# kyutai-labs/pocket-tts

Measured on AMD Instinct MI355X. Metric: audio-seconds/sec (xRT), 100M en model, whole job over all GPUs, higher is better.
Workload: dtype f32

## Files before the change

include/ptts.h:

```cpp
#ifndef PTTS_H_
#define PTTS_H_

#include <stdint.h>

#ifdef __cplusplus
extern "C" {
#endif

#define PTTS_ABI_VERSION 1

typedef struct ptts_engine ptts_engine;
typedef struct ptts_lm_state ptts_lm_state;
typedef struct ptts_mimi_state ptts_mimi_state;
typedef struct ptts_graph ptts_graph;
typedef struct ptts_resampler ptts_resampler;
typedef struct ptts_stretcher ptts_stretcher;
typedef struct ptts_pitcher ptts_pitcher;
typedef struct ptts_leveler ptts_leveler;
typedef struct ptts_loudnorm ptts_loudnorm;
typedef struct ptts_tone ptts_tone;
typedef struct ptts_dynamics ptts_dynamics;
typedef struct ptts_encoder ptts_encoder;
typedef struct ptts_flac ptts_flac;

// ... 39 lines not shown
int ptts_lm_state_copy(ptts_lm_state *dst, const ptts_lm_state *src, void *stream);
int ptts_lm_state_copy_row(ptts_lm_state *dst, int32_t row, const ptts_lm_state *src, void *stream);
int ptts_lm_state_copy_row_from(ptts_lm_state *dst, int32_t row, const ptts_lm_state *src, int32_t src_row, void *stream);
int ptts_lm_state_offsets(ptts_lm_state *s, int32_t *h_offsets, void *stream);

int ptts_lm_prefill(ptts_engine *e, ptts_lm_state *s, const float *d_emb, int32_t t, void *stream);
int ptts_lm_prefill_ragged(ptts_engine *e, ptts_lm_state *s, const float *d_emb, const int32_t *h_len, int32_t t_max,
                           void *stream);
int ptts_embed_tokens(ptts_engine *e, const float *d_table, int32_t n_bins, const int64_t *d_tokens, int64_t n,
                      float *d_out, void *stream);

int ptts_lm_decode_step(ptts_engine *e, ptts_lm_state *s, const float *d_latent_in, const float *d_noise,
                        int32_t lsd_steps, float eos_threshold, float *d_latent_out, float *d_eos_logit,
                        uint8_t *d_is_eos, void *stream);
int ptts_lm_set_noise(ptts_lm_state *s, float temp, uint64_t seed);
int ptts_lm_state_set_row_seed(ptts_lm_state *s, int32_t row, uint64_t seed, void *stream);
int ptts_lm_state_clear_row_seed(ptts_lm_state *s, int32_t row, void *stream);
int ptts_lm_state_set_row_sampling(ptts_lm_state *s, int32_t row, float temp, float noise_clamp, float eos_threshold,
                                   void *stream);
int ptts_lm_state_clear_row_sampling(ptts_lm_state *s, int32_t row, void *stream);
int ptts_lm_state_reserve_row_lsd(ptts_lm_state *s, int32_t K, void *stream);
int ptts_lm_state_set_row_lsd(ptts_lm_state *s, int32_t row, int32_t n, void *stream);
int ptts_lm_state_clear_row_lsd(ptts_lm_state *s, int32_t row, void *stream);
const float *ptts_lm_latent_ptr(ptts_lm_state *s);

int ptts_mimi_state_create(ptts_engine *e, int32_t batch, ptts_mimi_state **out);
void ptts_mimi_state_destroy(ptts_mimi_state *s);
int ptts_mimi_state_reset(ptts_mimi_state *s, void *stream);
int ptts_mimi_state_reset_row(ptts_mimi_state *s, int32_t row, void *stream);
int ptts_lm_state_set_row_active(ptts_lm_state *s, int32_t row, int32_t active, void *stream);
int ptts_mimi_set_pcm_i16(ptts_mimi_state *s, int16_t *d_pcm_i16);
int ptts_resampler_create(ptts_engine *e, int32_t batch, const int32_t *h_up, const int32_t *h_down, const int32_t *h_taps,
                          int32_t n_rates, const float *h_tables, int64_t n_table_floats, ptts_resampler **out);
void ptts_resampler_destroy(ptts_resampler *rs);
int ptts_resampler_set_row(ptts_resampler *rs, int32_t row, int32_t rate_index, void *stream);
int ptts_resample_frame(ptts_resampler *rs, const float *d_pcm_in, void *out, int32_t is_i16, void *stream);
int ptts_mimi_set_resampler(ptts_mimi_state *s, ptts_resampler *rs, void *out, int32_t is_i16);
int ptts_stretcher_create(ptts_engine *e, int32_t batch, const int32_t *h_plans, int32_t n_plans, const float *h_windows,
                          int64_t n_window_floats, ptts_stretcher **out);
void ptts_stretcher_destroy(ptts_stretcher *ts);
int ptts_stretcher_set_row(ptts_stretcher *ts, int32_t row, int32_t plan_index, void *stream);
int ptts_stretcher_set_row_drain(ptts_stretcher *ts, int32_t row, int32_t on, void *stream);
int ptts_stretch_frame(ptts_stretcher *ts, const float *d_in, void *out, int32_t is_i16, int32_t *d_delta, void *stream);
int ptts_mimi_set_stretcher(ptts_mimi_state *s, ptts_stretcher *ts, float *d_in, void *out, int32_t is_i16);
int ptts_pitcher_create(ptts_engine *e, int32_t batch, const int32_t *h_plans, int32_t n_plans, const float *h_windows,
                        int64_t n_window_floats, const float *h_tables, int64_t n_table_floats, ptts_pitcher **out);
// ... 158 lines not shown
```

pocket_tts_amd/_lib.py:

```python

from __future__ import annotations

import ctypes as C
import os
import subprocess
from pathlib import Path

PKG = Path(__file__).resolve().parent
LIB_PATH = PKG / "libptts.so"
SRC = PKG / "csrc" / "ptts.hip"
HEADER = PKG.parent / "include" / "ptts.h"

HIPCC_FLAGS = ["--offload-arch=gfx950", "-O3", "-std=c++17", "-ffp-contract=on", "-Wno-unused-value", "-Wno-unused-result",
               "-shared", "-fPIC"]


class PttsConfig(C.Structure):
    _fields_ = [
        ("d_model", C.c_int32), ("num_heads", C.c_int32), ("num_layers", C.c_int32), ("ff_dim", C.c_int32),
        ("ldim", C.c_int32), ("flow_dim", C.c_int32), ("flow_depth", C.c_int32), ("max_period", C.c_float),
        ("m_dim", C.c_int32), ("m_heads", C.c_int32), ("m_layers", C.c_int32), ("m_ff", C.c_int32),
        ("m_context", C.c_int32), ("m_max_period", C.c_float),
        ("n_filters", C.c_int32), ("ratios", C.c_int32 * 3), ("kernel_size", C.c_int32),
        ("res_kernel_size", C.c_int32), ("last_kernel_size", C.c_int32), ("compress", C.c_int32),
# ... 46 lines not shown
    "ptts_create_from_file": (C.c_int, [C.c_char_p, C.c_int32, C.POINTER(_P)]),
    "ptts_destroy": (None, [_P]),
    "ptts_lm_state_create": (C.c_int, [_P, C.c_int32, C.c_int32, C.POINTER(_P)]),
    "ptts_lm_state_destroy": (None, [_P]),
    "ptts_lm_state_reset": (C.c_int, [_P, _P]),
    "ptts_lm_state_import": (C.c_int, [_P, C.c_int32, _P, C.c_int32, C.c_int32, _P]),
    "ptts_lm_state_export": (C.c_int, [_P, C.c_int32, _P, C.c_int32, _P]),
    "ptts_lm_state_copy": (C.c_int, [_P, _P, _P]),
    "ptts_lm_state_copy_row": (C.c_int, [_P, C.c_int32, _P, _P]),
    "ptts_lm_state_copy_row_from": (C.c_int, [_P, C.c_int32, _P, C.c_int32, _P]),
    "ptts_lm_state_offsets": (C.c_int, [_P, C.POINTER(C.c_int32), _P]),
    "ptts_lm_prefill": (C.c_int, [_P, _P, _P, C.c_int32, _P]),
    "ptts_lm_prefill_ragged": (C.c_int, [_P, _P, _P, _P, C.c_int32, _P]),
    "ptts_lm_decode_step": (C.c_int, [_P, _P, _P, _P, C.c_int32, C.c_float, _P, _P, _P, _P]),
    "ptts_lm_latent_ptr": (_P, [_P]),
    "ptts_lm_set_noise": (C.c_int, [_P, C.c_float, C.c_uint64]),
    "ptts_lm_state_set_row_sampling": (C.c_int, [_P, C.c_int32, C.c_float, C.c_float, C.c_float, _P]),
    "ptts_lm_state_clear_row_sampling": (C.c_int, [_P, C.c_int32, _P]),
    "ptts_lm_state_set_row_seed": (C.c_int, [_P, C.c_int32, C.c_uint64, _P]),
    "ptts_lm_state_clear_row_seed": (C.c_int, [_P, C.c_int32, _P]),
    "ptts_lm_state_reserve_row_lsd": (C.c_int, [_P, C.c_int32, _P]),
    "ptts_lm_state_set_row_lsd": (C.c_int, [_P, C.c_int32, C.c_int32, _P]),
    "ptts_lm_state_clear_row_lsd": (C.c_int, [_P, C.c_int32, _P]),
    "ptts_profile_start": (C.c_int, [_P]),
    "ptts_profile_stop": (C.c_int64, [_P, C.c_char_p, C.c_int64]),
    "ptts_mimi_state_create": (C.c_int, [_P, C.c_int32, C.POINTER(_P)]),
    "ptts_mimi_state_destroy": (None, [_P]),
    "ptts_mimi_state_reset": (C.c_int, [_P, _P]),
    "ptts_mimi_decode": (C.c_int, [_P, _P, _P, _P, _P]),
    "ptts_encode_voice": (C.c_int, [_P, _P, C.c_int64, _P, _P, C.POINTER(C.c_int32), _P]),
    "ptts_graph_capture_lm_step": (C.c_int, [_P, _P, _P, C.c_int32, C.c_float, _P, _P, _P, C.POINTER(_P)]),
    "ptts_graph_capture_mimi": (C.c_int, [_P, _P, _P, _P, C.POINTER(_P)]),
    "ptts_mimi_decode_tr": (C.c_int, [_P, _P, _P, _P, _P]),
    "ptts_mimi_decode_seanet": (C.c_int, [_P, _P, _P, _P]),
    "ptts_graph_capture_mimi_tr": (C.c_int, [_P, _P, _P, C.POINTER(_P)]),
    "ptts_graph_capture_mimi_tr_pair": (C.c_int, [_P, _P, _P, _P, C.POINTER(_P)]),
    "ptts_graph_capture_mimi_seanet": (C.c_int, [_P, _P, _P, C.POINTER(_P)]),
    "ptts_graph_capture_pipelined": (C.c_int, [_P, _P, _P, _P, C.c_int32, C.c_float, _P, _P, _P, _P, _P, C.POINTER(_P)]),
    "ptts_graph_launch": (C.c_int, [_P, _P]),
    "ptts_graph_destroy": (None, [_P]),
    "ptts_mimi_state_reset_row": (C.c_int, [_P, C.c_int32, _P]),
    "ptts_lm_state_set_row_active": (C.c_int, [_P, C.c_int32, C.c_int32, _P]),
    "ptts_mimi_set_pcm_i16": (C.c_int, [_P, _P]),
    "ptts_resampler_create": (C.c_int, [_P, C.c_int32, C.POINTER(C.c_int32), C.POINTER(C.c_int32), C.POINTER(C.c_int32),
                                        C.c_int32, C.POINTER(C.c_float), C.c_int64, C.POINTER(_P)]),
    "ptts_resampler_destroy": (None, [_P]),
# ... 162 lines not shown
```

pocket_tts_amd/csrc/ptts.hip:

```cpp
#include "ptts_host.h"
#include "ptts_flow.h"
#include "ptts_bf16.h"
#include "ptts_lm.h"

#include <algorithm>
#include <array>
#include <cmath>
#include <cstdio>
#include <cstring>

static thread_local std::string g_err;
int fail(int code, const std::string &msg) {
  g_err = msg;
  return code;
}
static thread_local std::string g_launch_err;
bool launch_err_pending() { return !g_launch_err.empty(); }
int take_launch_err() {
  std::string m;
  m.swap(g_launch_err);
  return fail(-4, m);
}
void note_launch_err(const std::string &msg) { if (g_launch_err.empty()) g_launch_err = msg; }

// ... 1097 lines not shown
  hipStream_t st = S(s->e, stream);
  ENGINE_LOCK(s->e);
  set_int_kernel<<<1, 64, 0, st>>>(s->seed_on + row, 1, 0);
  LAUNCHCHK();
  return 0;
}

static int ensure_flow(ptts_engine *e, ptts_lm_state *s, int steps, hipStream_t st);

extern "C" int ptts_lm_state_reserve_row_lsd(ptts_lm_state *s, int32_t K, void *stream) {
  if (!s || K < 1 || K > 64) return fail(-1, "reserve_row_lsd: capacity must be in [1, 64]");
  ptts_engine *e = s->e;
  ENGINE_LOCK(e);
  HIPCHK(hipSetDevice(e->device));
  if (s->n_graphs > 0) return fail(-1, "reserve_row_lsd: the state has captured graphs (they hold its flow buffers): reserve before capturing");
  K = std::max(K, (int32_t)s->lsd_cap);
  CHK(ensure_flow(e, s, K, S(e, stream)));
  CHK(prepare_lsd_pack(e, K));
  s->lsd_tab = e->tpack[K];
  s->lsd_cap = K;
  return 0;
}

extern "C" int ptts_lm_state_set_row_lsd(ptts_lm_state *s, int32_t row, int32_t n, void *stream) {
  if (!s || row < 0 || row >= s->B) return fail(-1, "set_row_lsd: row out of range");
  if (s->lsd_cap < 1) return fail(-1, "set_row_lsd: the state has no per-row LSD capacity (ptts_lm_state_reserve_row_lsd)");
  if (n < 1 || n > s->lsd_cap) return fail(-1, "set_row_lsd: lsd_decode_steps must be in [1, " + std::to_string(s->lsd_cap) + "]");
  hipStream_t st = S(s->e, stream);
  ENGINE_LOCK(s->e);
  set_int_kernel<<<1, 64, 0, st>>>(s->lsd_n + row, 1, n);
  LAUNCHCHK();
  return 0;
}

extern "C" int ptts_lm_state_clear_row_lsd(ptts_lm_state *s, int32_t row, void *stream) {
  if (!s || row < 0 || row >= s->B) return fail(-1, "clear_row_lsd: row out of range");
  hipStream_t st = S(s->e, stream);
  ENGINE_LOCK(s->e);
  set_int_kernel<<<1, 64, 0, st>>>(s->lsd_n + row, 1, 0);
  LAUNCHCHK();
  return 0;
}

extern "C" int ptts_profile_start(ptts_engine *e) {
  if (!e) return fail(-1, "null engine");
  ENGINE_LOCK(e);
// ... 22 lines not shown
  e->prof.recs.clear();
  std::string out;
  char line[512];
  for (auto &k : order) {
    auto &v = agg[k];
    snprintf(line, sizeof line, "%s %s %.0f %.6f %.0f %.0f\n", k.first.empty() ? "-" : k.first.c_str(), k.second.c_str(), v[0], v[1], v[2], v[3]);
    out += line;
  }
  if ((int64_t)out.size() + 1 > capacity) return fail(-1, "profile buffer too small");
  memcpy(h_out, out.c_str(), out.size() + 1);
  return (int64_t)out.size();
}


static bool flow_cluster_ok(const ptts_engine *e, const ptts_lm_state *s) {
  const ptts_config &c = e->cfg;
  const int FDF = c.flow_dim / 16, LF = c.ldim / 16;
  if (!e->opt_flow_cluster || c.flow_depth > FLOW_MAX_DEPTH || FDF > 64 || LF > FDF) return false;
  const int kpw = cdiv(std::max(FDF, LF), FLOW_WORKERS);
  if (kpw != 1 && kpw != 2 && kpw != 4) return false;
  if (!e->input_proj.bias || !e->fin.bias) return false;
  for (auto &r : e->res) if (!r.l0.bias || !r.l2.bias) return false;
  return FDF <= std::min(e->opt_flow_max_cus, e->n_cus);
}
static int ensure_flow(ptts_engine *e, ptts_lm_state *s, int steps, hipStream_t st) {
  if (steps <= s->flow_steps) return 0;
  if (s->n_graphs > 0)
    return fail(-1, "lsd_decode_steps grows beyond what this state's captured graphs were built for: destroy the graphs first "
                    "(they hold the old AdaLN / exchange buffers)");
  const ptts_config &c = e->cfg;
  const int FDF = c.flow_dim / 16;
  static const int rt_env = [] { const char *v = getenv("PTTS_FLOW_RT"); return v ? atoi(v) : 1; }();
  s->flow_rt = (rt_env == 2 && s->MT >= 2) ? 2 : 1;
  s->flow_ng = cdiv(s->MT, s->flow_rt);
  HIPCHK(hipStreamSynchronize(st));
  HIPCHK(hipStreamSynchronize(e->stream));
  AllocScope alloc_scope(st);
  hipFree(s->mod); hipFree(s->fexch); hipFree(s->fflags);
  s->mod = nullptr; s->fexch = nullptr; s->fflags = nullptr;
  const size_t rt = (size_t)s->MT * 256;
  const int nph = steps * (2 * c.flow_depth + 2);
  CHK(dallocT(nullptr, &s->mod, (size_t)steps * rt * e->adaln.NT));
  CHK(dallocT(nullptr, &s->fexch, (size_t)s->flow_ng * nph * s->flow_rt * FDF * 256));
  CHK(dallocT(nullptr, &s->fflags, (size_t)s->flow_ng * nph * FDF));
  HIPCHK(hipStreamSynchronize(st));
  s->flow_steps = steps;
  return 0;
}

template <int RT, bool ROWLSD>
static void launch_flow_rt(hipStream_t st, const FlowArgs &fa, int kpw) {
  const dim3 grid(fa.NCL * fa.FDF), block(FLOW_THREADS);
  switch (kpw) {
    case 1: flow_cluster_kernel<RT, 1, ROWLSD><<<grid, block, 0, st>>>(fa); break;
    case 2: flow_cluster_kernel<RT, 2, ROWLSD><<<grid, block, 0, st>>>(fa); break;
    default: flow_cluster_kernel<RT, 4, ROWLSD><<<grid, block, 0, st>>>(fa); break;
  }
}

static int flow_steps_of(const ptts_lm_state *s, int lsd_steps) { return std::max(lsd_steps, s->lsd_cap); }

static void launch_flow_cluster(hipStream_t st, ptts_engine *e, ptts_lm_state *s, int lsd_steps, float *d_latent_out) {
  const ptts_config &c = e->cfg;
  const int FDF = c.flow_dim / 16, LF = c.ldim / 16;
  FlowArgs fa;
  memset(&fa, 0, sizeof fa);
  fa.MT = s->MT; fa.M = s->B; fa.NG = s->flow_ng; fa.NCL = std::max(1, std::min(s->flow_ng, std::min(e->opt_flow_max_cus, e->n_cus) / FDF)); fa.FDF = FDF; fa.LF = LF; fa.AF = e->adaln.NT;
  const bool rowlsd = s->lsd_cap > 0;
  fa.depth = c.flow_depth; fa.steps = rowlsd ? flow_steps_of(s, lsd_steps) : lsd_steps; fa.ldim = c.ldim;
  fa.w_in = e->input_proj.w; fa.b_in = e->input_proj.bias;
  for (int r = 0; r < c.flow_depth; ++r) {
    fa.w_l0[r] = e->res[r].l0.w; fa.b_l0[r] = e->res[r].l0.bias;
    fa.w_l2[r] = e->res[r].l2.w; fa.b_l2[r] = e->res[r].l2.bias;
    fa.ln_w[r] = e->res[r].ln_w; fa.ln_b[r] = e->res[r].ln_b;
  }
  fa.w_fin = e->fin.w; fa.b_fin = e->fin.bias;
  fa.mod = s->mod; fa.mod_step = (long)s->MT * 256 * e->adaln.NT;
  fa.latfm = s->latfm;
  fa.lat = s->lat; fa.lat_out1 = s->lat_prev; fa.lat_out2 = d_latent_out;
  fa.inv_steps = 1.0f / (float)lsd_steps;
  fa.exch = s->fexch; fa.flags = s->fflags; fa.ctr = s->rng_ctr; fa.err = s->ferr;
  fa.row_n = rowlsd ? s->lsd_n : nullptr; fa.row_ndef = lsd_steps;
  const double wbytes = 4.0 * 256 * ((double)FDF * LF + 2.0 * c.flow_depth * FDF * FDF + (double)LF * FDF);
  const double flops = 2.0 * s->B * 256.0 * ((double)FDF * LF + 2.0 * c.flow_depth * FDF * FDF + (double)LF * FDF) * lsd_steps;
  ProfScope ps(st, std::string(rowlsd ? "flow_cluster_rowlsd@" : "flow_cluster@") + std::to_string((long)fa.NCL * FDF * FLOW_THREADS),
               lsd_steps * (wbytes + 4.0 * s->B * 16.0 * e->adaln.NT), flops);
  const int kpw = cdiv(std::max(FDF, LF), FLOW_WORKERS);
  s->coop_wgs = std::max(s->coop_wgs, fa.NCL * FDF);
  if (rowlsd) {
    if (s->flow_rt == 2) launch_flow_rt<2, true>(st, fa, kpw);
    else launch_flow_rt<1, true>(st, fa, kpw);
  } else {
    if (s->flow_rt == 2) launch_flow_rt<2, false>(st, fa, kpw);
    else launch_flow_rt<1, false>(st, fa, kpw);
  }
}


static constexpr int kLmMaxWGs = 256;
static bool lm_cluster_ok(const ptts_engine *e, const ptts_lm_state *s) {
  if (!e->opt_lm_cluster || !e->lm_table) return false;
  if (e->cfg.d_model / 16 > std::min(kLmMaxWGs, e->n_cus)) return false;
  if (s->n_pre > 0) return false;
  return (double)s->kv_plane() * 4.0 < 2.0e9;
}
static int ensure_lm_cluster(ptts_engine *e, ptts_lm_state *s, hipStream_t st) {
  if (s->lexch || !e->lm_table) return 0;
  const ptts_config &c = e->cfg;
  const int DF = c.d_model / 16, FFF = c.ff_dim / 16;
  AllocScope alloc_scope(st);
  CHK(dallocT(nullptr, &s->lexch, (size_t)s->MT * c.num_layers * (4 * DF + FFF) * 256));
// ... 205 lines not shown
  GemmArgs a;
  if (lm_cluster_ok(e, s) && s->lexch) {
    SITE("lm.cluster");
    launch_lm_cluster(st, e, s, sc);
  } else {
    lm_layers(st, e, s, sc, B, 1, true);
  }
  SITE("flow.head");
  a = mk_gemm(e->head, sc.x, DF, MT, B);
  a.epi = EPI_HEAD; a.Y = s->ce; a.YF = FDF; a.head_nt = FDF; a.eos_thr = eos_thr;
  a.eos_on = s->samp_on; a.eos_row = s->samp_eos;
  a.eos_logit = s->eos_logit; a.is_eos = s->is_eos;
  a.eos_logit2 = d_eos_logit; a.is_eos2 = d_is_eos;
  a.tail_offset = s->offset; a.tail_ctr = s->rng_ctr; a.tail_rctr = s->seed_ctr; a.tail_active = s->active;
  const bool silu_in_head = lsd_steps == 1 && s->lsd_cap == 0;
  if (silu_in_head) { a.act = ACT_SILU; a.prevec = tcomb; }
  launch_gemm(st, a, PRE_LNFOLD);
  const int AF = e->adaln.NT;
  const bool rowlsd = s->lsd_cap > 0;
  const int nit = rowlsd ? flow_steps_of(s, lsd_steps) : lsd_steps;
  auto row_lsd = [&](GemmArgs &g, int i) {
    g.row_n = s->lsd_n; g.row_tab = s->lsd_tab; g.row_ndef = lsd_steps; g.row_i = i;
  };
  if (flow_cluster_ok(e, s) && nit <= s->flow_steps) {
    if (rowlsd) {
      SITE("flow.adaln");
      a = mk_gemm(e->adaln, s->ce, FDF, MT, B);
      a.prevec = tcomb; a.Y = s->mod; a.YF = AF;
      row_lsd(a, 0);
      a.row_nz = nit; a.row_zstride = (long)MT * 256 * AF;
      launch_gemm(st, a, PRE_ADDSILU_ROW);
    } else {
      for (int i = 0; i < lsd_steps; ++i) {
        SITE("flow.adaln");
        a = mk_gemm(e->adaln, s->ce, FDF, MT, B);
        a.prevec = tcomb + (size_t)i * FD; a.Y = s->mod + (size_t)i * MT * 256 * AF; a.YF = AF;
        launch_gemm(st, a, silu_in_head ? PRE_NONE : PRE_ADDSILU);
      }
    }
    SITE("flow.cluster");
    launch_flow_cluster(st, e, s, lsd_steps, d_latent_out);
    s->latfm_noise = true;
  } else {
  s->latfm_noise = false;
  for (int i = 0; i < nit; ++i) {
    SITE("flow.adaln");
    a = mk_gemm(e->adaln, s->ce, FDF, MT, B);
// ... 434 lines not shown
```

pocket_tts_amd/csrc/ptts_debug.hip:

```cpp
#include "ptts_bf16.h"
#include "ptts_host.h"

#include <algorithm>
#include <cstring>


static constexpr unsigned kDbgUnwritten = 0x7fc00000u;
static constexpr unsigned kDbgGuard = 0x7fa5a5a5u;
static constexpr long kDbgGuardFloats = 16384;
static constexpr long kAttnGuard = 16 * 64;

static __global__ void dbg_guard_kernel(const unsigned *p, long n, unsigned pattern, int *bad) {
  const long i = (long)blockIdx.x * blockDim.x + threadIdx.x;
  if (i < n && p[i] != pattern) atomicOr(bad, 1);
}
__device__ __forceinline__ float dbg_e4m3(uint8_t b) { return __builtin_amdgcn_cvt_f32_fp8((int)b, 0); }
static __global__ void dbg_from_codec_kernel(const void *src, float *dst, int M, int N, int KB, int fmt) {
  const long i = (long)blockIdx.x * blockDim.x + threadIdx.x;
  if (i >= (long)M * N) return;
  const int m = i / N, n = i - (long)m * N;
  const size_t o = fmh_off(m, n & ~3, KB) + (n & 3);
  dst[i] = fmt == 0 ? (float)((const __bf16 *)src)[o] : dbg_e4m3(((const uint8_t *)src)[o]);
}

// ... 22 lines not shown
  int *bad = nullptr;
  CHK(dallocT(&scr, &bad, 1));
  for (const void *g : guards) dbg_guard_kernel<<<cdiv(n, 256), 256, 0, st>>>((const unsigned *)g, n, kDbgGuard, bad);
  LAUNCHCHK();
  int h_bad = 0;
  HIPCHK(hipMemcpyAsync(&h_bad, bad, sizeof(int), hipMemcpyDeviceToHost, st));
  HIPCHK(hipStreamSynchronize(st));
  if (h_bad) return fail(-6, what);
  return 0;
}

extern "C" int64_t ptts_debug_read(ptts_engine *e, void *state, int32_t is_mimi, const char *name, float *d_out,
                                   int64_t capacity, int32_t *rows, int32_t *cols, void *stream) {
  hipStream_t st = S(e, stream);
  const ptts_config &c = e->cfg;
  const float *src = nullptr;
  int M = 0, K = 0, F = 0;
  std::string n(name);
  if (!is_mimi) {
    ptts_lm_state *s = (ptts_lm_state *)state;
    if (n == "x") { src = s->dec.x; M = s->B; K = c.d_model; }
    else if (n == "ce") { src = s->ce; M = s->B; K = c.flow_dim; }
    else if (n == "fx") { src = s->fx; M = s->B; K = c.flow_dim; }
    else if (n == "prefill_x") { src = s->pre.x; M = s->pre.MT * 16; K = c.d_model; }
    else if (n == "noise") {
      if (!s->latfm_noise) return fail(-1, "debug_read: noise is only kept by steps that ran the flow cluster");
      src = s->latfm; M = s->B; K = c.ldim;
    }
    else return fail(-1, "unknown buffer " + n);
    F = K / 16;
  } else {
    ptts_mimi_state *s = (ptts_mimi_state *)state;
    const int par = (s->h_frame - 1) & 1;
    const int B = s->B;
    if (n == "upsample") { src = s->u0; M = B * 16; K = c.m_dim; }
    else if (n == "dec_tr") { src = s->tr_out.slot((s->h_frame - 1) & (s->tr_out.slots - 1)); M = B * 16; K = c.m_dim; }
    else if (n.compare(0, 11, "dec_tr_slot") == 0) {
      const int k = atoi(n.c_str() + 11);
      if (n.size() != 12 || k < 0 || k >= s->tr_out.slots) return fail(-1, "unknown buffer " + n);
      src = s->tr_out.slot(k); M = B * 16; K = c.m_dim;
    }
    else if (n == "seanet0") { src = s->a0.slot(par); M = B * 16; K = 8 * c.n_filters; }
    else if (n == "tr_attn") { src = s->ao; M = B * 16; K = c.m_dim; }
    else if (n == "tr_resid") { src = s->u; M = B * 16; K = c.m_dim; }
    else if (n == "tr_ff") { src = s->ff; M = B * 16; K = c.m_ff; }
    else if (n == "seanet11") {
// ... 586 lines not shown
```

pocket_tts_amd/csrc/ptts_flow.h:

```cpp
#pragma once
#include "ptts_kernels.h"

#define FLOW_MAX_DEPTH 12
#define FLOW_WORKERS 8
#define FLOW_THREADS (64 * (FLOW_WORKERS + 1))
#define FLOW_SPIN_LIMIT 400000u

typedef unsigned u32x4 __attribute__((ext_vector_type(4)));
typedef unsigned long long u64;

struct FlowArgs {
  int MT, M, NG, NCL, FDF, LF, AF, depth, steps, ldim;
  const float *w_in, *b_in;
  const float *w_l0[FLOW_MAX_DEPTH], *b_l0[FLOW_MAX_DEPTH], *w_l2[FLOW_MAX_DEPTH], *b_l2[FLOW_MAX_DEPTH];
  const float *ln_w[FLOW_MAX_DEPTH], *ln_b[FLOW_MAX_DEPTH];
  const float *w_fin, *b_fin;
  const float *mod;
  long mod_step;
  const float *latfm;
  float *lat, *lat_out1, *lat_out2;
  float inv_steps;
  float *exch;
  u64 *flags;
  const int *ctr;
  int *err;
  const int *row_n;
  int row_ndef;
};

__device__ __forceinline__ __amdgpu_buffer_rsrc_t flow_rsrc(const void *p) {
  return __builtin_amdgcn_make_buffer_rsrc(const_cast<void *>(p), 0, 0x7ffffff0, 0x00020000);
}
__device__ __forceinline__ f32x4 flow_ld_sc1(__amdgpu_buffer_rsrc_t r, unsigned byte_off) {
  return __builtin_bit_cast(f32x4, __builtin_amdgcn_raw_buffer_load_b128(r, (int)byte_off, 0, 16));
}
__device__ __forceinline__ void flow_st_sc1(__amdgpu_buffer_rsrc_t r, unsigned byte_off, f32x4 v) {
  __builtin_amdgcn_raw_buffer_store_b128(__builtin_bit_cast(u32x4, v), r, (int)byte_off, 0, 16);
}

__device__ __forceinline__ bool flow_wait(const u64 *f, int np, u64 epoch, int lane, int *err) {
  for (unsigned spins = 0;; ++spins) {
    const u64 v = lane < np ? __hip_atomic_load(f + lane, __ATOMIC_RELAXED, __HIP_MEMORY_SCOPE_AGENT) : epoch;
    if (__all(v == epoch)) return true;
    if (spins > FLOW_SPIN_LIMIT) {
      if (lane == 0) atomicExch(err, 1);
      return false;
    }
    __builtin_amdgcn_s_sleep(2);
  }
}

template <int RT, int KPW, bool ROWLSD = false>
__global__ __launch_bounds__(FLOW_THREADS) void flow_cluster_kernel(FlowArgs a) {
  const int lane = threadIdx.x & 63, wave = threadIdx.x >> 6;
  const int FDF = a.FDF, LF = a.LF;
  const int cl = blockIdx.x / a.FDF, j = blockIdx.x % a.FDF;
  const bool coord = wave == FLOW_WORKERS;
  const int PPS = 2 * a.depth + 2, NPH = a.steps * PPS;
  __shared__ f32x4 red[FLOW_WORKERS][RT][64];
  __shared__ float st[FLOW_WORKERS][RT][16][2];
// ... 202 lines not shown
          latv[t] = latv[t] + s * a.inv_steps;
        }
        out = latv[t];
        const int m = 16 * (mt0 + t) + (lane & 15);
        if (last && j < LF && mt0 + t < a.MT && m < a.M) {
          const size_t o = (size_t)m * a.ldim + 16 * j + 4 * (lane >> 4);
          *(f32x4 *)(a.lat + o) = out;
          if (a.lat_out1) *(f32x4 *)(a.lat_out1 + o) = out;
          if (a.lat_out2) *(f32x4 *)(a.lat_out2 + o) = out;
        }
      }
      if (publish) flow_st_sc1(rs, ((unsigned)((p * RT + t) * FDF + j) * 64u + lane) * 16u, out);
    }
    if (publish) {
      asm volatile("s_waitcnt vmcnt(0)" ::: "memory");
      if (lane == 0) __hip_atomic_store(fl + (size_t)p * FDF + j, ebase | (u64)(p + 1), __ATOMIC_RELAXED, __HIP_MEMORY_SCOPE_AGENT);
    }
    e_bias = n_bias;
#pragma unroll
    for (int t = 0; t < RT; ++t) e_gate[t] = n_gate[t];
  }
  }
}
```

pocket_tts_amd/csrc/ptts_host.h:

```cpp
#pragma once
#include "ptts_kernels.h"
#include "ptts_ext.h"

#include <array>
#include <map>
#include <mutex>
#include <string>
#include <vector>

#include "../../include/ptts.h"

#pragma GCC visibility push(hidden)

int fail(int code, const std::string &msg);
#define HIPCHK(x)                                                                                      \
  do {                                                                                                 \
    hipError_t e_ = (x);                                                                               \
    if (e_ != hipSuccess)                                                                              \
      return fail(-2, std::string(#x) + ": " + hipGetErrorString(e_) + " @" + std::to_string(__LINE__)); \
  } while (0)
#define CHK(x)            \
  do {                    \
    int r_ = (x);         \
    if (r_ < 0) return r_; \
// ... 121 lines not shown
  int quant_flags = 0;
};
#define ENGINE_LOCK(e) std::lock_guard<std::recursive_mutex> lock_((e)->mu)

struct Scratch {
  float *x = nullptr, *h = nullptr, *ao = nullptr, *ff = nullptr, *q = nullptr, *part = nullptr, *rope = nullptr;
  int MT = 0, QB = 0, splits_cap = 0;
};

struct ptts_lm_state {
  ptts_engine *e;
  int B, cap, MT;
  float *kv = nullptr;
  int *offset = nullptr;
  int *qlen = nullptr;
  std::vector<int> h_off;
  Scratch dec, pre;
  float *xlat, *c, *ce, *mod, *latfm, *fx, *fh, *f1;
  float *fstat = nullptr;
  float *fexch = nullptr;
  unsigned long long *fflags = nullptr;
  int *ferr = nullptr;
  int flow_steps = 0, flow_rt = 1, flow_ng = 1;
  int lsd_cap = 0;
  const float *lsd_tab = nullptr;
  int *lsd_n = nullptr;
  KvPrefix *d_pre = nullptr;
  std::vector<KvPrefix> h_pre;
  std::vector<ptts_lm_state *> pre_owner;
  int casc_mode = -1;
  int n_pre = 0;
  int borrowers = 0;
  bool zombie = false;
  int n_graphs = 0;
  int coop_wgs = 0;
  float *lexch = nullptr;
  unsigned long long *lflags = nullptr;
  float *lat, *lat_prev;
  float *eos_logit;
  uint8_t *is_eos;
  float rng_std = 0.f;
  unsigned long long rng_seed = 0;
  int *rng_ctr = nullptr;
  int *samp_on = nullptr;
  f32x4 *samp_noise = nullptr;
  float *samp_eos = nullptr;
// ... 138 lines not shown
```

pocket_tts_amd/engine.py:

```python

from __future__ import annotations

import ctypes as C
import numbers
import os
import weakref

import numpy as np
import torch

from . import _lib
from .config import Config
from .weights import mimi_encode_spec, state_dict_spec


def _ptr(t: torch.Tensor | None):
    return None if t is None else C.c_void_p(t.data_ptr())


def make_ptts_config(cfg: Config) -> _lib.PttsConfig:
    t, m, sn = cfg.flow_lm.transformer, cfg.mimi.transformer, cfg.mimi.seanet
    if len(sn.ratios) != 3:
        raise ValueError("SEANet decoder with 3 upsampling stages expected")
    pc = _lib.PttsConfig()
# ... 71 lines not shown
    def set_row_sampling(self, row: int, temp: float, noise_clamp: float | None = None, eos_threshold: float = -4.0):
        clamp = 0.0 if noise_clamp is None else float(noise_clamp)
        _lib.check(self.engine.lib.ptts_lm_state_set_row_sampling(self.handle, row, float(temp), clamp,
                                                                  float(eos_threshold), self.engine._sp))

    def clear_row_sampling(self, row: int):
        _lib.check(self.engine.lib.ptts_lm_state_clear_row_sampling(self.handle, row, self.engine._sp))

    def set_row_seed(self, row: int, seed: int):
        _lib.check(self.engine.lib.ptts_lm_state_set_row_seed(self.handle, row, check_seed(seed, bits=64),
                                                              self.engine._sp))

    def clear_row_seed(self, row: int):
        _lib.check(self.engine.lib.ptts_lm_state_clear_row_seed(self.handle, row, self.engine._sp))

    def reserve_row_lsd(self, K: int):
        _lib.check(self.engine.lib.ptts_lm_state_reserve_row_lsd(self.handle, int(K), self.engine._sp))

    def set_row_lsd(self, row: int, n: int):
        _lib.check(self.engine.lib.ptts_lm_state_set_row_lsd(self.handle, row, int(n), self.engine._sp))

    def clear_row_lsd(self, row: int):
        _lib.check(self.engine.lib.ptts_lm_state_clear_row_lsd(self.handle, row, self.engine._sp))

    def error(self) -> bool:
        r = self.engine.lib.ptts_lm_state_error(self.handle, self.engine._sp)
        _lib.check(min(int(r), 0))
        return bool(r)

    def offsets(self) -> np.ndarray:
        out = (C.c_int32 * self.batch)()
        _lib.check(self.engine.lib.ptts_lm_state_offsets(self.handle, out, self.engine._sp))
        return np.array(out[:], dtype=np.int64)

    def import_layer(self, layer: int, cache: torch.Tensor, t: int):
        e = self.engine
        if cache.dim() != 5 or cache.shape[0] != 2 or cache.shape[1] not in (1, self.batch) or cache.shape[2] < t \
                or cache.shape[3] != e.H or cache.shape[4] != 64:
            raise ValueError(f"voice-state cache of layer {layer}: expected [2, 1|{self.batch}, >={t}, {e.H}, 64], "
                             f"got {tuple(cache.shape)}")
        cache = cache[:, :, :t].to(self.engine.device, torch.float32).contiguous()
        self.engine._pre()
        _lib.check(self.engine.lib.ptts_lm_state_import(self.handle, layer, _ptr(cache), cache.shape[1], t, self.engine._sp))
        self.engine.sync()

    def export_layer(self, layer: int, t: int) -> torch.Tensor:
# ... 1095 lines not shown
        out["splits"] = c.splits_used
        return out

    def close(self):
        if self.handle is not None:
            for st in list(self._states):
                st.close()
            self.lib.ptts_destroy(self.handle)
            self.handle = None

    def __del__(self):
        try:
            self.close()
        except Exception:
            pass


class StepPipeline:

    NB_EVENTS = int(os.environ.get("PTTS_PIPE_NB", "4"))

    def __init__(self, eng: Engine, lm_state: LMState, mimi_state: MimiState, noise=None, lsd_steps: int = 1,
                 eos_threshold: float = -4.0, mode: str | None = None, pcm_i16: bool = False,
                 lm_stream: torch.cuda.Stream | None = None, spec=None, codec_pair: bool | None = None, **chain):
        from .output_chain import ChainSpec, OutputChain

        self.eng, self.st, self.ms = eng, lm_state, mimi_state
        B, dev = lm_state.batch, eng.device
        self.mode = mode or ("hostsync" if B <= 8 else "events")
        if codec_pair is None:
            codec_pair = os.environ.get("PTTS_CODEC_PAIR", "1") != "0" and B > 8
        self.codec_pair = bool(codec_pair) and self.mode == "events" and not (
            {"codec_bf16", "codec_fp8"} & set(eng.quantize_groups))
        table = ChainSpec.of(spec, **chain).table(eng.sample_rate, eng.frame_samples)
        if not table.empty and self.mode == "fork":
            raise ValueError("sample_rates / speeds / pitches / tones / dynamics / loudness / level / encodings: not available in the "
                             "'fork' mode")
        self.nb = nb = self.NB_EVENTS if self.mode == "events" else 2
        self.chain = OutputChain(eng, B, table, nb, pcm_i16)
        self.out = self.chain.out
        self.rs, self.ts, self.ps, self.tn, self.dy, self.ln, self.lv, self.en = self.chain.per_kind()
        self.pk = self.chain.pk
        self.lat = [torch.zeros(B, eng.ldim, device=dev) for _ in range(nb)]
        self.logit = [torch.empty(B, device=dev) for _ in range(nb)]
        self.flag = [torch.zeros(B, dtype=torch.uint8).pin_memory() for _ in range(nb)]
        self.pcm = [torch.zeros(B, eng.frame_samples, device=dev) if self.out is not None else
                    torch.zeros(B, eng.frame_samples).pin_memory() for _ in range(nb)]
        self.ev = [torch.cuda.Event() for _ in range(nb)]
        self.ev_lm = [torch.cuda.Event() for _ in range(nb)]
        self.s1 = lm_stream or eng.stream
        self.s2 = eng.concurrent_stream(self.s1)
        eng.sync()
        torch.cuda.synchronize(dev)
        eng.tune(B)
        lib, H = eng.lib, eng.handle
        self.g_first = [eng.capture_lm_step(lm_state, noise, lsd_steps, eos_threshold, self.lat[p], self.logit[p],
                                            self.flag[p]) for p in range(nb)]
        self.pcm16 = [torch.zeros(B, eng.frame_samples, dtype=torch.int16).pin_memory() for _ in range(nb)] \
            if pcm_i16 and self.out is None else None
        self.g_last, self.g_sn, self.g_tr1, self.g_tr2 = [], [], [], []
        for p in range(nb):
            if self.out is not None:
                self.chain.attach(mimi_state, p)
            else:
                mimi_state.set_pcm_i16(self.pcm16[p] if pcm_i16 else None)
            self.g_last.append(eng.capture_mimi(mimi_state, self.lat[p], self.pcm[p]))
            if self.codec_pair:
                self.g_sn.append(eng.capture_mimi_seanet(mimi_state, self.pcm[p]))
                self.g_tr1.append(eng.capture_mimi_tr(mimi_state, self.lat[p]))
                self.g_tr2.append(eng.capture_mimi_tr(mimi_state, self.lat[(p - 1) % nb], self.lat[p]))
        mimi_state.set_pcm_i16(None)
        self.chain.detach(mimi_state)
        self.g_both = []
        if self.mode == "fork":
            for p in range(nb):
                g = C.c_void_p()
                _lib.check(lib.ptts_graph_capture_pipelined(
                    H, lm_state.handle, mimi_state.handle, _ptr(noise), lsd_steps, eos_threshold, _ptr(self.lat[p]),
# ... 136 lines not shown
```

Measured before the change: 6105.

## Fold AdaLN modulation GEMM into the flow cluster kernel

Adds a flow_cluster_mod_kernel that computes the AdaLN modulation (shift/scale/gate) inside the persistent flow cluster. Each phase computes only the modulation tiles it needs from the conditioning embedding and exchanges them through an enlarged per-phase exchange buffer. This replaces the separate adaln GEMM and the full mod tensor write/read. The pipeline turns it on by default for batches above 8 in events mode. In exchange each cluster step does extra MFMA work and weight loads, adds more exchange traffic and barriers, and the mod tensor is no longer materialised for debugging.

```diff
diff --git a/include/ptts.h b/include/ptts.h
--- a/include/ptts.h
+++ b/include/ptts.h
@@ -85,6 +85,10 @@
 int ptts_lm_state_reserve_row_lsd(ptts_lm_state *s, int32_t K, void *stream);
 int ptts_lm_state_set_row_lsd(ptts_lm_state *s, int32_t row, int32_t n, void *stream);
 int ptts_lm_state_clear_row_lsd(ptts_lm_state *s, int32_t row, void *stream);
+int ptts_lm_state_set_flow_fold(ptts_lm_state *s, int32_t on, void *stream);
+int64_t ptts_flow_slot_offset(int32_t fdf, int32_t rt, int32_t nph, int32_t nf, int32_t grp, int32_t p, int32_t t, int32_t j,
+                              int32_t f);
+int32_t ptts_flow_mod_tiles(int32_t fdf, int32_t depth, int32_t ph, int32_t j, int32_t *n);
 const float *ptts_lm_latent_ptr(ptts_lm_state *s);
 
 int ptts_mimi_state_create(ptts_engine *e, int32_t batch, ptts_mimi_state **out);
diff --git a/pocket_tts_amd/_lib.py b/pocket_tts_amd/_lib.py
--- a/pocket_tts_amd/_lib.py
+++ b/pocket_tts_amd/_lib.py
@@ -92,6 +92,9 @@
     "ptts_lm_state_reserve_row_lsd": (C.c_int, [_P, C.c_int32, _P]),
     "ptts_lm_state_set_row_lsd": (C.c_int, [_P, C.c_int32, C.c_int32, _P]),
     "ptts_lm_state_clear_row_lsd": (C.c_int, [_P, C.c_int32, _P]),
+    "ptts_lm_state_set_flow_fold": (C.c_int, [_P, C.c_int32, _P]),
+    "ptts_flow_slot_offset": (C.c_int64, [C.c_int32] * 9),
+    "ptts_flow_mod_tiles": (C.c_int32, [C.c_int32, C.c_int32, C.c_int32, C.c_int32, C.POINTER(C.c_int32)]),
     "ptts_profile_start": (C.c_int, [_P]),
     "ptts_profile_stop": (C.c_int64, [_P, C.c_char_p, C.c_int64]),
     "ptts_mimi_state_create": (C.c_int, [_P, C.c_int32, C.POINTER(_P)]),
diff --git a/pocket_tts_amd/csrc/ptts.hip b/pocket_tts_amd/csrc/ptts.hip
--- a/pocket_tts_amd/csrc/ptts.hip
+++ b/pocket_tts_amd/csrc/ptts.hip
@@ -1143,6 +1143,31 @@
   return 0;
 }
 
+extern "C" int ptts_lm_state_set_flow_fold(ptts_lm_state *s, int32_t on, void *stream) {
+  if (!s) return fail(-1, "set_flow_fold: null state");
+  ptts_engine *e = s->e;
+  ENGINE_LOCK(e);
+  HIPCHK(hipSetDevice(e->device));
+  if ((on != 0) == s->flow_fold) return 0;
+  if (s->n_graphs > 0) return fail(-1, "set_flow_fold: the state has captured graphs (they hold its flow buffers): set it before capturing");
+  const int steps = s->flow_steps;
+  s->flow_fold = on != 0;
+  s->flow_steps = 0;
+  return ensure_flow(e, s, std::max(1, steps), S(e, stream));
+}
+
+extern "C" int64_t ptts_flow_slot_offset(int32_t fdf, int32_t rt, int32_t nph, int32_t nf, int32_t grp, int32_t p, int32_t t,
+                                         int32_t j, int32_t f) {
+  return (int64_t)flow_slot(fdf, rt, nph, nf, grp, p, t, j, f);
+}
+
+extern "C" int32_t ptts_flow_mod_tiles(int32_t fdf, int32_t depth, int32_t ph, int32_t j, int32_t *n) {
+  int nn = 0;
+  const int t0 = flow_mod_tiles(fdf, depth, ph, j, &nn);
+  if (n) *n = nn;
+  return t0;
+}
+
 extern "C" int ptts_lm_state_set_row_lsd(ptts_lm_state *s, int32_t row, int32_t n, void *stream) {
   if (!s || row < 0 || row >= s->B) return fail(-1, "set_row_lsd: row out of range");
   if (s->lsd_cap < 1) return fail(-1, "set_row_lsd: the state has no per-row LSD capacity (ptts_lm_state_reserve_row_lsd)");
@@ -1211,6 +1236,12 @@
   if (!e->input_proj.bias || !e->fin.bias) return false;
   for (auto &r : e->res) if (!r.l0.bias || !r.l2.bias) return false;
   return FDF <= std::min(e->opt_flow_max_cus, e->n_cus);
+}
+static bool flow_fold_ok(const ptts_engine *e, const ptts_lm_state *s) {
+  const int FDF = e->cfg.flow_dim / 16;
+  const Lin &m = e->adaln;
+  return s->flow_fold && flow_cluster_ok(e, s) && s->lsd_cap == 0 && s->flow_rt == 1 && m.w && m.bias && !m.wq && !m.wb16 &&
+         m.KF == FDF && m.NT == (3 * e->cfg.flow_depth + 2) * FDF;
 }
 static int ensure_flow(ptts_engine *e, ptts_lm_state *s, int steps, hipStream_t st) {
   if (steps <= s->flow_steps) return 0;
@@ -1230,7 +1261,7 @@
   const size_t rt = (size_t)s->MT * 256;
   const int nph = steps * (2 * c.flow_depth + 2);
   CHK(dallocT(nullptr, &s->mod, (size_t)steps * rt * e->adaln.NT));
-  CHK(dallocT(nullptr, &s->fexch, (size_t)s->flow_ng * nph * s->flow_rt * FDF * 256));
+  CHK(dallocT(nullptr, &s->fexch, flow_slot(FDF, s->flow_rt, nph, s->flow_fold ? FLOW_MOD_FRAGS : 1, s->flow_ng, 0, 0, 0, 0)));
   CHK(dallocT(nullptr, &s->fflags, (size_t)s->flow_ng * nph * FDF));
   HIPCHK(hipStreamSynchronize(st));
   s->flow_steps = steps;
@@ -1249,7 +1280,8 @@
 
 static int flow_steps_of(const ptts_lm_state *s, int lsd_steps) { return std::max(lsd_steps, s->lsd_cap); }
 
-static void launch_flow_cluster(hipStream_t st, ptts_engine *e, ptts_lm_state *s, int lsd_steps, float *d_latent_out) {
+static void launch_flow_cluster(hipStream_t st, ptts_engine *e, ptts_lm_state *s, int lsd_steps, float *d_latent_out,
+                                bool fold = false, const float *tcomb = nullptr, bool ce_silu = false) {
   const ptts_config &c = e->cfg;
   const int FDF = c.flow_dim / 16, LF = c.ldim / 16;
   FlowArgs fa;
@@ -1270,12 +1302,22 @@
   fa.inv_steps = 1.0f / (float)lsd_steps;
   fa.exch = s->fexch; fa.flags = s->fflags; fa.ctr = s->rng_ctr; fa.err = s->ferr;
   fa.row_n = rowlsd ? s->lsd_n : nullptr; fa.row_ndef = lsd_steps;
-  const double wbytes = 4.0 * 256 * ((double)FDF * LF + 2.0 * c.flow_depth * FDF * FDF + (double)LF * FDF);
-  const double flops = 2.0 * s->B * 256.0 * ((double)FDF * LF + 2.0 * c.flow_depth * FDF * FDF + (double)LF * FDF) * lsd_steps;
-  ProfScope ps(st, std::string(rowlsd ? "flow_cluster_rowlsd@" : "flow_cluster@") + std::to_string((long)fa.NCL * FDF * FLOW_THREADS),
-               lsd_steps * (wbytes + 4.0 * s->B * 16.0 * e->adaln.NT), flops);
+  if (fold) { fa.mod = nullptr; fa.ce = s->ce; fa.w_mod = e->adaln.w; fa.b_mod = e->adaln.bias; fa.tcomb = tcomb; fa.ce_silu = ce_silu; }
+  const double wbytes = 4.0 * 256 * ((double)FDF * LF + 2.0 * c.flow_depth * FDF * FDF + (double)LF * FDF + (fold ? (double)e->adaln.NT * FDF : 0.0));
+  const double flops = 2.0 * s->B * 256.0 * ((double)FDF * LF + 2.0 * c.flow_depth * FDF * FDF + (double)LF * FDF + (fold ? (double)e->adaln.NT * FDF : 0.0)) * lsd_steps;
+  ProfScope ps(st, std::string(fold ? "flow_cluster_mod@" : rowlsd ? "flow_cluster_rowlsd@" : "flow_cluster@") + std::to_string((long)fa.NCL * FDF * FLOW_THREADS),
+               lsd_steps * (wbytes + 4.0 * s->B * 16.0 * (fold ? FDF : e->adaln.NT)), flops);
   const int kpw = cdiv(std::max(FDF, LF), FLOW_WORKERS);
   s->coop_wgs = std::max(s->coop_wgs, fa.NCL * FDF);
+  if (fold) {
+    const dim3 grid(fa.NCL * fa.FDF), block(FLOW_THREADS);
+    switch (kpw) {
+      case 1: flow_cluster_mod_kernel<1><<<grid, block, 0, st>>>(fa); break;
+      case 2: flow_cluster_mod_kernel<2><<<grid, block, 0, st>>>(fa); break;
+      default: flow_cluster_mod_kernel<4><<<grid, block, 0, st>>>(fa); break;
+    }
+    return;
+  }
   if (rowlsd) {
     if (s->flow_rt == 2) launch_flow_rt<2, true>(st, fa, kpw);
     else launch_flow_rt<1, true>(st, fa, kpw);
@@ -1527,7 +1569,13 @@
   auto row_lsd = [&](GemmArgs &g, int i) {
     g.row_n = s->lsd_n; g.row_tab = s->lsd_tab; g.row_ndef = lsd_steps; g.row_i = i;
   };
-  if (flow_cluster_ok(e, s) && nit <= s->flow_steps) {
+  s->mod_stale = false;
+  if (flow_fold_ok(e, s) && nit <= s->flow_steps) {
+    SITE("flow.cluster");
+    launch_flow_cluster(st, e, s, lsd_steps, d_latent_out, true, tcomb, silu_in_head);
+    s->latfm_noise = true;
+    s->mod_stale = true;
+  } else if (flow_cluster_ok(e, s) && nit <= s->flow_steps) {
     if (rowlsd) {
       SITE("flow.adaln");
       a = mk_gemm(e->adaln, s->ce, FDF, MT, B);
diff --git a/pocket_tts_amd/csrc/ptts_debug.hip b/pocket_tts_amd/csrc/ptts_debug.hip
--- a/pocket_tts_amd/csrc/ptts_debug.hip
+++ b/pocket_tts_amd/csrc/ptts_debug.hip
@@ -68,6 +68,11 @@
     if (n == "x") { src = s->dec.x; M = s->B; K = c.d_model; }
     else if (n == "ce") { src = s->ce; M = s->B; K = c.flow_dim; }
     else if (n == "fx") { src = s->fx; M = s->B; K = c.flow_dim; }
+    else if (n == "mod") {
+      if (s->mod_stale) return fail(-1, "debug_read: mod is not materialised by a step with the flow fold (ptts_lm_state_set_flow_fold): the cluster computes it on chip");
+      if (!s->mod) return fail(-1, "debug_read: mod is not allocated");
+      src = s->mod; M = s->B; K = e->adaln.NT * 16;
+    }
     else if (n == "prefill_x") { src = s->pre.x; M = s->pre.MT * 16; K = c.d_model; }
     else if (n == "noise") {
       if (!s->latfm_noise) return fail(-1, "debug_read: noise is only kept by steps that ran the flow cluster");
diff --git a/pocket_tts_amd/csrc/ptts_flow.h b/pocket_tts_amd/csrc/ptts_flow.h
--- a/pocket_tts_amd/csrc/ptts_flow.h
+++ b/pocket_tts_amd/csrc/ptts_flow.h
@@ -26,7 +26,24 @@
   int *err;
   const int *row_n;
   int row_ndef;
+  const float *ce, *w_mod, *b_mod;
+  const float *tcomb;
+  int ce_silu;
 };
+
+#define FLOW_MOD_FRAGS 3
+__host__ __device__ inline size_t flow_slot(int FDF, int RT, int NPH, int nf, int grp, int p, int t, int j, int f) {
+  return ((((((size_t)grp * NPH + p) * RT + t) * FDF + j) * nf) + f) * 256;
+}
+
+__host__ __device__ inline int flow_mod_tiles(int FDF, int depth, int ph, int j, int *n) {
+  const int r = (ph - 1) >> 1;
+  if (ph == 0) { *n = 2; return j; }
+  if (ph == 2 * depth + 1) { *n = 0; return 0; }
+  if ((ph - 1) & 1) { *n = 2; return (r + 1) * 3 * FDF + j; }
+  *n = 1;
+  return r * 3 * FDF + 2 * FDF + j;
+}
 
 __device__ __forceinline__ __amdgpu_buffer_rsrc_t flow_rsrc(const void *p) {
   return __builtin_amdgcn_make_buffer_rsrc(const_cast<void *>(p), 0, 0x7ffffff0, 0x00020000);
@@ -36,6 +53,16 @@
 }
 __device__ __forceinline__ void flow_st_sc1(__amdgpu_buffer_rsrc_t r, unsigned byte_off, f32x4 v) {
   __builtin_amdgcn_raw_buffer_store_b128(__builtin_bit_cast(u32x4, v), r, (int)byte_off, 0, 16);
+}
+
+__device__ __forceinline__ f32x4 flow_ldu(const void *base, unsigned voff) {
+  return __builtin_bit_cast(f32x4, __builtin_amdgcn_raw_buffer_load_b128(flow_rsrc(base), (int)voff, 0, 0));
+}
+__device__ __forceinline__ f32x4 flow_ldu_sc1(__amdgpu_buffer_rsrc_t r, unsigned soff, unsigned voff) {
+  return __builtin_bit_cast(f32x4, __builtin_amdgcn_raw_buffer_load_b128(r, (int)voff, (int)soff, 16));
+}
+__device__ __forceinline__ void flow_stu_sc1(__amdgpu_buffer_rsrc_t r, unsigned soff, unsigned voff, f32x4 v) {
+  __builtin_amdgcn_raw_buffer_store_b128(__builtin_bit_cast(u32x4, v), r, (int)voff, (int)soff, 16);
 }
 
 __device__ __forceinline__ bool flow_wait(const u64 *f, int np, u64 epoch, int lane, int *err) {
@@ -284,3 +311,245 @@
   }
   }
 }
+
+template <int KPW>
+__global__ __launch_bounds__(FLOW_THREADS) void flow_cluster_mod_kernel(FlowArgs a) {
+  const int lane = threadIdx.x & 63, wave = __builtin_amdgcn_readfirstlane(threadIdx.x >> 6);
+  const int FDF = a.FDF, LF = a.LF;
+  const int cl = blockIdx.x / a.FDF, j = blockIdx.x % a.FDF;
+  const bool coord = wave == FLOW_WORKERS;
+  const int PPS = 2 * a.depth + 2, NPH = a.steps * PPS;
+  __shared__ f32x4 red[FLOW_WORKERS][64];
+  __shared__ f32x4 mred[FLOW_WORKERS][2][64];
+  __shared__ f32x4 cxs[FLOW_WORKERS][KPW][64];
+  __shared__ float st[FLOW_WORKERS][16][2];
+  const u64 ebase = ((u64)(unsigned)(*a.ctr) + 1ull) << 16;
+  const f32x4 zero4 = {0.f, 0.f, 0.f, 0.f};
+  bool dead = false;
+  auto slot = [&](int p, int q, int f) { return (unsigned)flow_slot(FDF, 1, NPH, FLOW_MOD_FRAGS, 0, p, 0, q, f) * 4u; };
+  const unsigned l16 = (unsigned)lane * 16u, q16 = (unsigned)(lane >> 4) * 16u;
+  for (int grp = cl; grp < a.NG; grp += a.NCL) {
+  float *ex = a.exch + flow_slot(FDF, 1, NPH, FLOW_MOD_FRAGS, grp, 0, 0, 0, 0);
+  u64 *fl = a.flags + (size_t)grp * NPH * FDF;
+  const __amdgpu_buffer_rsrc_t rs = flow_rsrc(ex);
+  __syncthreads();
+  const int mtc = min(grp, a.MT - 1);
+  const int nph = NPH;
+
+  auto kind_of = [&](int ph) { return ph == 0 ? 0 : ph == PPS - 1 ? 3 : 1 + ((ph - 1) & 1); };
+  auto wtile = [&](int ph, int &KF, bool &use) -> const float * {
+    const int k = kind_of(ph), r = (ph - 1) >> 1;
+    use = true;
+    if (k == 0) { KF = LF; return a.w_in + (size_t)j * LF * 256; }
+    KF = FDF;
+    if (k == 1) return a.w_l0[r] + (size_t)j * FDF * 256;
+    if (k == 2) return a.w_l2[r] + (size_t)j * FDF * 256;
+    use = j < LF;
+    return a.w_fin + (size_t)(use ? j : 0) * FDF * 256;
+  };
+  auto bias_of = [&](int ph) -> const float * {
+    const int k = kind_of(ph), r = (ph - 1) >> 1;
+    return (k == 0 ? a.b_in : k == 1 ? a.b_l0[r] : k == 2 ? a.b_l2[r] : a.b_fin) + (k == 3 && j >= LF ? 0 : 16 * j);
+  };
+  auto mtiles = [&](int ph, int &n) { return flow_mod_tiles(FDF, a.depth, ph, j, &n); };
+
+  f32x4 w[KPW], mw[2][KPW];
+  auto load_w = [&](int ph) {
+    int n;
+    const int t0 = mtiles(ph, n);
+#pragma unroll
+    for (int s = 0; s < 2; ++s) {
+#pragma unroll
+      for (int u = 0; u < KPW; ++u) mw[s][u] = zero4;
+      if (s < n) {
+#pragma unroll
+        for (int u = 0; u < KPW; ++u) {
+          const int kf = wave * KPW + u;
+          const f32x4 v = flow_ldu(a.w_mod + ((size_t)(t0 + s * FDF) * FDF + min(kf, FDF - 1)) * 256, l16);
+          if (kf < FDF) mw[s][u] = v;
+        }
+      }
+    }
+    int KF;
+    bool use;
+    const float *Wt = wtile(ph, KF, use);
+#pragma unroll
+    for (int u = 0; u < KPW; ++u) {
+      const int kf = wave * KPW + u;
+      const f32x4 v = flow_ldu(Wt + (size_t)min(kf, KF - 1) * 256, l16);
+      w[u] = (use && kf < KF) ? v : zero4;
+    }
+  };
+  if (coord) {
+    f32x4 xres = zero4, latv = zero4, e_gate = zero4;
+    if (j < LF) latv = flow_ldu(a.latfm + ((size_t)mtc * LF + j) * 256, l16);
+    for (int p = 0; p < nph; ++p) {
+      const int i = p / PPS, ph = p - i * PPS;
+      const int kind = kind_of(ph);
+      const bool lnmod = kind == 1 || kind == 3;
+      int nmt;
+      const int t0 = mtiles(ph, nmt);
+      const f32x4 e_bias = flow_ldu(bias_of(ph), q16);
+      f32x4 mbias[2] = {zero4, zero4};
+#pragma unroll
+      for (int s = 0; s < 2; ++s)
+        if (s < nmt) mbias[s] = flow_ldu(a.b_mod + 16 * (t0 + s * FDF), q16);
+      if (p > 0 && !dead) {
+        const int np = ph == 0 ? LF : FDF;
+        if (!flow_wait(fl + (size_t)(p - 1) * FDF, np, ebase | (u64)p, lane, a.err)) dead = true;
+      }
+      __syncthreads();
+      if (nmt > 0) {
+        auto msum = [&](int s) {
+          f32x4 m = mred[0][s][lane];
+#pragma unroll
+          for (int q = 1; q < FLOW_WORKERS; ++q) m += mred[q][s][lane];
+          return m + mbias[s];
+        };
+        const f32x4 m0 = msum(0);
+        if (nmt == 2) {
+          flow_stu_sc1(rs, slot(p, j, 1), l16, m0);
+          flow_stu_sc1(rs, slot(p, j, 2), l16, msum(1));
+        } else {
+          e_gate = m0;
+        }
+      }
+      if (lnmod) __syncthreads();
+      __syncthreads();
+      const bool publish = p + 1 < nph && (kind != 3 || j < LF);
+      f32x4 s = red[0][lane];
+#pragma unroll
+      for (int q = 1; q < FLOW_WORKERS; ++q) s += red[q][lane];
+      s += e_bias;
+      f32x4 out;
+      if (kind == 0) { xres = s; out = s; }
+      else if (kind == 1) out = act4(s, ACT_SILU);
+      else if (kind == 2) { xres = xres + e_gate * s; out = xres; }
+      else {
+        latv = latv + s * a.inv_steps;
+        out = latv;
+        const int m = 16 * grp + (lane & 15);
+        if (i == a.steps - 1 && j < LF && m < a.M) {
+          const size_t o = (size_t)m * a.ldim + 16 * j + 4 * (lane >> 4);
+          *(f32x4 *)(a.lat + o) = out;
+          if (a.lat_out1) *(f32x4 *)(a.lat_out1 + o) = out;
+          if (a.lat_out2) *(f32x4 *)(a.lat_out2 + o) = out;
+        }
+      }
+      if (publish) {
+        flow_stu_sc1(rs, slot(p, j, 0), l16, out);
+        asm volatile("s_waitcnt vmcnt(0)" ::: "memory");
+        if (lane == 0) __hip_atomic_store(fl + (size_t)p * FDF + j, ebase | (u64)(p + 1), __ATOMIC_RELAXED, __HIP_MEMORY_SCOPE_AGENT);
+      }
+    }
+  } else {
+    load_w(0);
+    for (int p = 0; p < nph; ++p) {
+      const int i = p / PPS, ph = p - i * PPS;
+      const int kind = kind_of(ph);
+      const int KF = kind == 0 ? LF : FDF;
+      const bool lnmod = kind == 1 || kind == 3;
+      int nmt;
+      mtiles(ph, nmt);
+      if (ph == 0) {
+#pragma unroll
+        for (int u = 0; u < KPW; ++u) {
+          const int kf = wave * KPW + u, kc = min(kf, FDF - 1);
+          f32x4 v = flow_ldu(a.ce + ((size_t)mtc * FDF + kc) * 256, l16);
+          if (!a.ce_silu) {
+            const f32x4 t = flow_ldu(a.tcomb + (size_t)i * FDF * 16 + 16 * kc, q16);
+            v.x = silu_f(v.x + t.x); v.y = silu_f(v.y + t.y); v.z = silu_f(v.z + t.z); v.w = silu_f(v.w + t.w);
+          }
+          cxs[wave][u][lane] = kf < FDF ? v : zero4;
+        }
+      }
+      if (nmt > 0) {
+        f32x4 m0 = zero4, m1 = zero4, cx[KPW];
+#pragma unroll
+        for (int u = 0; u < KPW; ++u) cx[u] = cxs[wave][u][lane];
+#pragma unroll
+        for (int u = 0; u < KPW; ++u)
+#pragma unroll
+          for (int c = 0; c < 4; ++c) m0 = __builtin_amdgcn_mfma_f32_16x16x4f32(mw[0][u][c], cx[u][c], m0, 0, 0, 0);
+        mred[wave][0][lane] = m0;
+        if (nmt == 2) {
+#pragma unroll
+          for (int u = 0; u < KPW; ++u)
+#pragma unroll
+            for (int c = 0; c < 4; ++c) m1 = __builtin_amdgcn_mfma_f32_16x16x4f32(mw[1][u][c], cx[u][c], m1, 0, 0, 0);
+          mred[wave][1][lane] = m1;
+        }
+      }
+      __syncthreads();
+      f32x4 x[KPW], ma[KPW], mb[KPW];
+      const int r = (ph - 1) >> 1;
+      if (p == 0) {
+#pragma unroll
+        for (int u = 0; u < KPW; ++u) {
+          const int kf = wave * KPW + u;
+          const f32x4 v = flow_ldu(a.latfm + ((size_t)mtc * LF + min(kf, KF - 1)) * 256, l16);
+          x[u] = kf < KF ? v : zero4;
+        }
+      } else {
+#pragma unroll
+        for (int u = 0; u < KPW; ++u) {
+          const int kf = wave * KPW + u;
+          const f32x4 v = flow_ldu_sc1(rs, slot(p - 1, min(kf, KF - 1), 0), l16);
+          x[u] = kf < KF ? v : zero4;
+        }
+      }
+      if (lnmod) {
+#pragma unroll
+        for (int u = 0; u < KPW; ++u) {
+          const int kf = min(wave * KPW + u, KF - 1);
+          f32x4 lw = {1.f, 1.f, 1.f, 1.f}, lb = zero4;
+          if (kind == 1) {
+            lw = flow_ldu(a.ln_w[r] + 16 * kf, q16);
+            lb = flow_ldu(a.ln_b[r] + 16 * kf, q16);
+          }
+          const f32x4 shv = flow_ldu_sc1(rs, slot(p - 1, kf, 1), l16), scv = 1.0f + flow_ldu_sc1(rs, slot(p - 1, kf, 2), l16);
+          ma[u] = lw * scv;
+          mb[u] = lb * scv + shv;
+        }
+        float s1 = 0.f, s2 = 0.f;
+#pragma unroll
+        for (int u = 0; u < KPW; ++u) {
+          const f32x4 v = x[u];
+          s1 += (v.x + v.y) + (v.z + v.w);
+          s2 += (v.x * v.x + v.y * v.y) + (v.z * v.z + v.w * v.w);
+        }
+        s1 += __shfl_xor(s1, 16); s1 += __shfl_xor(s1, 32);
+        s2 += __shfl_xor(s2, 16); s2 += __shfl_xor(s2, 32);
+        if (lane < 16) { st[wave][lane][0] = s1; st[wave][lane][1] = s2; }
+      }
+      if (lnmod) __syncthreads();
+      if (lnmod) {
+        const float invK = 1.0f / (float)(KF * 16);
+        float t0 = 0.f, t1 = 0.f;
+#pragma unroll
+        for (int q = 0; q < FLOW_WORKERS; ++q) { t0 += st[q][lane & 15][0]; t1 += st[q][lane & 15][1]; }
+        const float mu = t0 * invK;
+        const float rsd = 1.0f / sqrtf(fmaxf(t1 * invK - mu * mu, 0.f) + 1e-6f);
+#pragma unroll
+        for (int u = 0; u < KPW; ++u) {
+          const f32x4 v = ((x[u] - mu) * rsd) * ma[u] + mb[u];
+          x[u] = (wave * KPW + u) < KF ? v : zero4;
+        }
+      }
+      f32x4 acc = zero4;
+#pragma unroll
+      for (int u = 0; u < KPW; ++u)
+#pragma unroll
+        for (int c = 0; c < 4; ++c) acc = __builtin_amdgcn_mfma_f32_16x16x4f32(w[u][c], x[u][c], acc, 0, 0, 0);
+      red[wave][lane] = acc;
+      __syncthreads();
+      if (p + 1 < nph) {
+        load_w((p + 1) % PPS);
+      } else {
+#pragma unroll
+        for (int u = 0; u < KPW; ++u) w[u] = mw[0][u] = mw[1][u] = zero4;
+      }
+    }
+  }
+  }
+}
diff --git a/pocket_tts_amd/csrc/ptts_host.h b/pocket_tts_amd/csrc/ptts_host.h
--- a/pocket_tts_amd/csrc/ptts_host.h
+++ b/pocket_tts_amd/csrc/ptts_host.h
@@ -167,6 +167,8 @@
   unsigned long long *fflags = nullptr;
   int *ferr = nullptr;
   int flow_steps = 0, flow_rt = 1, flow_ng = 1;
+  bool flow_fold = false;
+  bool mod_stale = false;
   int lsd_cap = 0;
   const float *lsd_tab = nullptr;
   int *lsd_n = nullptr;
diff --git a/pocket_tts_amd/engine.py b/pocket_tts_amd/engine.py
--- a/pocket_tts_amd/engine.py
+++ b/pocket_tts_amd/engine.py
@@ -117,6 +117,9 @@
 
     def clear_row_lsd(self, row: int):
         _lib.check(self.engine.lib.ptts_lm_state_clear_row_lsd(self.handle, row, self.engine._sp))
+
+    def set_flow_fold(self, on: bool):
+        _lib.check(self.engine.lib.ptts_lm_state_set_flow_fold(self.handle, int(bool(on)), self.engine._sp))
 
     def error(self) -> bool:
         r = self.engine.lib.ptts_lm_state_error(self.handle, self.engine._sp)
@@ -1258,7 +1261,8 @@
 
     def __init__(self, eng: Engine, lm_state: LMState, mimi_state: MimiState, noise=None, lsd_steps: int = 1,
                  eos_threshold: float = -4.0, mode: str | None = None, pcm_i16: bool = False,
-                 lm_stream: torch.cuda.Stream | None = None, spec=None, codec_pair: bool | None = None, **chain):
+                 lm_stream: torch.cuda.Stream | None = None, spec=None, codec_pair: bool | None = None, flow_fold: bool | None = None,
+                 **chain):
         from .output_chain import ChainSpec, OutputChain
 
         self.eng, self.st, self.ms = eng, lm_state, mimi_state
@@ -1268,6 +1272,10 @@
             codec_pair = os.environ.get("PTTS_CODEC_PAIR", "1") != "0" and B > 8
         self.codec_pair = bool(codec_pair) and self.mode == "events" and not (
             {"codec_bf16", "codec_fp8"} & set(eng.quantize_groups))
+        if flow_fold is None:
+            flow_fold = os.environ.get("PTTS_FLOW_FOLD", "1") != "0" and B > 8
+        self.flow_fold = bool(flow_fold) and self.mode == "events" and not (
+            {"lm_bf16", "attention", "ffn", "codec_split"} & set(eng.quantize_groups))
         table = ChainSpec.of(spec, **chain).table(eng.sample_rate, eng.frame_samples)
         if not table.empty and self.mode == "fork":
             raise ValueError("sample_rates / speeds / pitches / tones / dynamics / loudness / level / encodings: not available in the "
@@ -1290,6 +1298,11 @@
         torch.cuda.synchronize(dev)
         eng.tune(B)
         lib, H = eng.lib, eng.handle
+        if self.flow_fold:
+            try:
+                lm_state.set_flow_fold(True)
+            except _lib.PttsError:
+                self.flow_fold = False
         self.g_first = [eng.capture_lm_step(lm_state, noise, lsd_steps, eos_threshold, self.lat[p], self.logit[p],
                                             self.flag[p]) for p in range(nb)]
         self.pcm16 = [torch.zeros(B, eng.frame_samples, dtype=torch.int16).pin_memory() for _ in range(nb)] \
```

After: 6250 (median of 6 runs). +2.4%, better.
